# Herong1212/ORB_SLAM3_comments_ghr

Hardware: AMD Instinct MI355X
Metric: Mmatches/s (256-bit Hamming) (higher is better)
Workload: dtype fp4(e2m1)->f32; 1 GPU; C2: brute-force 256-bit Hamming top-2, 2000 x 2000 descriptors per frame, 1024 independent frames per launch per GPU (headline; the one-frame launch is `sing...; nq=2000, nt=2000, global_batch=1024, parallelism=replicas x1 (independent frames per GPU, no data-path collective)

## Files before the change

### orb_slam3_comments_ghr_amd/csrc/hamming_mfma.hip

```cpp
#include <algorithm>
#include <cstdlib>

#include "osg_internal.h"
#include "top2_key.h"

namespace {

typedef int i32x4 __attribute__((ext_vector_type(4)));
typedef int i32x16 __attribute__((ext_vector_type(16)));

constexpr int MF_PAD = 1 << 30;
constexpr int MF_RS = 272;

__device__ __forceinline__ int med3_i32(int a, int b, int c)
{
    return max(min(a, b), min(max(a, b), c));
}

__device__ __forceinline__ uint32_t spread_query(uint32_t nib)
{
    const uint32_t s = __umul24(nib, 0x204081u) & 0x01010101u;
    return ((0x80808080u - s) & 0x80808080u) | 0x40404040u;
}

__device__ __forceinline__ void key_push(int &k1, int &k2, int key)
{
    k2 = med3_i32(k1, key, k2);
    k1 = min(k1, key);
}

__device__ __forceinline__ void key_push2(int &k1, int &k2, int x, int y)
{
    const int m = med3_i32(k1, x, y);
    k1 = min(min(k1, x), y);
    k2 = min(m, k2);
}

__device__ __forceinline__ void key_push2f(int &k1, int &k2, int x, int y)
{
    const int m = __float_as_int(__builtin_amdgcn_fmed3f(__int_as_float(k1), __int_as_float(x), __int_as_float(y)));
    k1 = min(min(x, y), k1);
    k2 = min(m, k2);
}

__device__ __forceinline__ void key_merge(int &k1, int &k2, int a1, int a2)
{
    const int hi = max(k1, a1);
    k1 = min(k1, a1);
    k2 = min(min(k2, a2), hi);
}

template <int NW, int QT, int CR, int PIPE>
__global__ __launch_bounds__(NW * 64) void k_top2_mfma(const uint32_t *__restrict__ query, int nq,
                                                        const uint32_t *__restrict__ train, int nt,
                                                        int nqb, int32_t *__restrict__ out)
{
    constexpr int NT = NW * 64;
    constexpr int BPT = CR * 32 / NT;
    constexpr int WPT = BPT / 4;
    constexpr int TPR = 32 / BPT;
    constexpr int NTILE = CR / 32;
    static_assert(CR * 32 % NT == 0 && BPT % 4 == 0 && TPR >= 1, "chunk / workgroup shape");
    __shared__ __attribute__((aligned(16))) unsigned char s_buf[2 * CR * MF_RS];
    __shared__ uint2 s_lut[256];

    const int t = threadIdx.x, lane = t & 63;
    const int w = __builtin_amdgcn_readfirstlane(t >> 6);
    const int G = gridDim.x, L = blockIdx.x;
    const int logical = (G % 8 == 0) ? (L % 8) * (G / 8) + L / 8 : L;
    const int b = logical / nqb, qb = logical % nqb;
    const uint32_t *qf = query + (size_t)b * nq * 8;
    const uint32_t *tf = train + (size_t)b * nt * 8;
    int32_t *of = out + (size_t)b * nq * 3;

    for (int e = t; e < 256; e += NT) {
        uint32_t lo = 0, hi = 0;
#pragma unroll
        for (int y = 0; y < 4; y++) {
            lo |= ((e >> y) & 1u) << (8 * y + 7);
            hi |= ((e >> (y + 4)) & 1u) << (8 * y + 7);
        }
        s_lut[e] = make_uint2(lo, hi);
    }

    const int r = lane & 31, h = lane >> 5;
    const int qw0 = qb * (NW * QT * 32) + w * (QT * 32);
    const bool active = qw0 < nq;

    i32x4 bq[QT][8];
    int ka1[QT], ka2[QT], kb1[QT], kb2[QT], pq[QT];
#pragma unroll
    for (int j = 0; j < QT; j++) {
        const int q = min(qw0 + 32 * j + r, nq - 1);
        const uint4 lo = *(const uint4 *)(qf + (size_t)q * 8), hi = *(const uint4 *)(qf + (size_t)q * 8 + 4);
        const uint32_t wd[8] = {lo.x, lo.y, lo.z, lo.w, hi.x, hi.y, hi.z, hi.w};
        int pc = 0;
#pragma unroll
        for (int s = 0; s < 8; s++) {
            pc += __popc(wd[s]);
            const uint32_t hw = h ? (wd[s] >> 16) : (wd[s] & 0xFFFFu);
#pragma unroll
            for (int d = 0; d < 4; d++) bq[j][s][d] = (int)spread_query((hw >> (4 * d)) & 0xFu);
        }
        pq[j] = pc;
        ka1[j] = ka2[j] = kb1[j] = kb2[j] = (256 - pc) << MF_SHIFT;
    }
    i32x16 crow;
#pragma unroll
    for (int i = 0; i < 16; i++) crow[i] = (i & 3) + 8 * (i >> 2) + 4 * h;
    const int lbase = r * MF_RS + h * 16;

    const int erow = t / TPR, epart = t % TPR;
    auto load_chunk = [&](int c0, uint32_t (&pw)[WPT]) {
        const int row = c0 + erow;
        if (row < nt) {
            const uint32_t *src = tf + (size_t)row * 8 + epart * WPT;
#pragma unroll
            for (int i = 0; i < WPT; i += 2) {
                const uint2 v = *(const uint2 *)(src + i);
                pw[i] = v.x;
                pw[i + 1] = v.y;
            }
        } else {
#pragma unroll
            for (int i = 0; i < WPT; i++) pw[i] = 0u;
        }
    };
    auto store_chunk = [&](int buf, const uint32_t (&pw)[WPT]) {
        unsigned char *dst = s_buf + ((size_t)buf * CR + erow) * MF_RS;
#pragma unroll
        for (int i = 0; i < WPT; i++) {
#pragma unroll
            for (int hh = 0; hh < 2; hh++) {
                const int g = 2 * (epart * WPT + i) + hh;
                const uint2 v0 = s_lut[(pw[i] >> (16 * hh)) & 0xFFu];
                const uint2 v1 = s_lut[(pw[i] >> (16 * hh + 8)) & 0xFFu];
                *(i32x4 *)(dst + 16 * g) = i32x4{(int)v0.x, (int)v0.y, (int)v1.x, (int)v1.y};
            }
        }
    };

    auto frag = [&](const unsigned char *tb, int s) -> i32x4 { return *(const i32x4 *)(tb + lbase + 32 * s); };
    auto mfma = [&](const i32x4 &a, const i32x4 &bb, const i32x16 &c) {
        return __builtin_amdgcn_mfma_i32_32x32x32_i8(a, bb, c, 0, 0, 0);
    };
    auto epi = [&](const i32x16 (&acc)[QT]) {
#pragma unroll
        for (int j = 0; j < QT; j++) {
#pragma unroll
            for (int i = 0; i < 8; i += 2) {
                key_push2(ka1[j], ka2[j], acc[j][i], acc[j][i + 1]);
                key_push2(kb1[j], kb2[j], acc[j][i + 8], acc[j][i + 9]);
            }
            ka1[j] -= 32;
            ka2[j] -= 32;
            kb1[j] -= 32;
            kb2[j] -= 32;
        }
    };
    auto tile = [&](const unsigned char *tb, const i32x16 &cin) {
        i32x4 a[8];
#pragma unroll
        for (int s = 0; s < 8; s++) a[s] = frag(tb, s);
        i32x16 acc[QT];
#pragma unroll
        for (int j = 0; j < QT; j++) acc[j] = mfma(a[0], bq[j][0], cin);
#pragma unroll
        for (int s = 1; s < 8; s++)
#pragma unroll
            for (int j = 0; j < QT; j++) acc[j] = mfma(a[s], bq[j][s], acc[j]);
        epi(acc);
    };

    const int nch = (nt + CR - 1) / CR;
    {
        uint32_t pw[WPT];
        load_chunk(0, pw);
        __syncthreads();
        store_chunk(0, pw);
    }
    __syncthreads();
    for (int c = 0; c < nch; c++) {
        const int c0 = c * CR;
        uint32_t pw[WPT];
        const bool more = c + 1 < nch;
        if (more) load_chunk(c0 + CR, pw);
        if (active) {
            const unsigned char *sb = s_buf + (size_t)(c & 1) * CR * MF_RS;
            const int nfull = min(NTILE, (nt - c0) / 32);
            if (PIPE && nfull == NTILE) {
                i32x4 a[8];
                i32x16 accp[QT], acc[QT];
#pragma unroll
                for (int s = 0; s < 8; s++) a[s] = frag(sb, s);
#pragma unroll
                for (int s = 0; s < 8; s++) {
#pragma unroll
                    for (int j = 0; j < QT; j++) accp[j] = mfma(a[s], bq[j][s], s ? accp[j] : crow);
                    a[s] = frag(sb + 32 * MF_RS, s);
                    __builtin_amdgcn_sched_barrier(0);
                }
#pragma unroll
                for (int tt = 1; tt < NTILE; tt++) {
#pragma unroll
                    for (int s = 0; s < 8; s++) {
#pragma unroll
                        for (int j = 0; j < QT; j++) acc[j] = mfma(a[s], bq[j][s], s ? acc[j] : crow);
                        if (tt + 1 < NTILE) a[s] = frag(sb + (tt + 1) * 32 * MF_RS, s);
#pragma unroll
                        for (int j = 0; j < QT; j++) {
                            if (s & 1)
                                key_push2(kb1[j], kb2[j], accp[j][8 + (s & 6)], accp[j][9 + (s & 6)]);
                            else
                                key_push2(ka1[j], ka2[j], accp[j][s & 6], accp[j][1 + (s & 6)]);
                            if (s == 7) {
                                ka1[j] -= 32;
                                ka2[j] -= 32;
                                kb1[j] -= 32;
                                kb2[j] -= 32;
                            }
                        }
                        __builtin_amdgcn_sched_barrier(0);
                    }
#pragma unroll
                    for (int j = 0; j < QT; j++) accp[j] = acc[j];
                }
                epi(accp);
            } else {
#pragma unroll
                for (int tt = 0; tt < NTILE; tt++) {
                    if (tt >= nfull) break;
                    tile(sb + tt * 32 * MF_RS, crow);
                }
            }
            const int lim = nt - (c0 + nfull * 32);
            if (nfull < NTILE && lim > 0) {
                i32x16 cin;
#pragma unroll
                for (int i = 0; i < 16; i++) cin[i] = crow[i] + (crow[i] >= lim ? MF_PAD : 0);
                tile(sb + nfull * 32 * MF_RS, cin);
            }
        }
        if (more) store_chunk((c + 1) & 1, pw);
        __syncthreads();
    }
    if (!active) return;
    const int base = 32 * ((nt + 31) / 32);
#pragma unroll
    for (int j = 0; j < QT; j++) {
        int k1 = ka1[j], k2 = ka2[j];
        key_merge(k1, k2, kb1[j], kb2[j]);
        const int a1 = __shfl_xor(k1, 32), a2 = __shfl_xor(k2, 32);
        key_merge(k1, k2, a1, a2);
        const int q = qw0 + 32 * j + r;
        if (h == 0 && q < nq) {
            const int t1 = k1 + base, t2 = k2 + base;
            const int d1 = (t1 >> MF_SHIFT) + pq[j], d2 = (t2 >> MF_SHIFT) + pq[j];
            of[3 * q + 0] = d1 < 256 ? (t1 & (MF_MAX_ROWS - 1)) : -1;
            of[3 * q + 1] = min(d1, 256);
            of[3 * q + 2] = min(d2, 256);
        }
    }
}

constexpr int MX_RS = 144;
constexpr int MX_SCALE_TRAIN = 127 + 12;
constexpr int MX_SCALE_ONE = 127;
constexpr float MX_BIAS = 10485760.0f;
constexpr float MX_PAD = 1073741824.0f;

typedef int i32x8 __attribute__((ext_vector_type(8)));
typedef float f32x16 __attribute__((ext_vector_type(16)));

__device__ __forceinline__ uint32_t spread_nib(uint32_t x)
{
    x &= 0xFFu;
    x = (x | (x << 12)) & 0x000F000Fu;
    x = (x | (x << 6)) & 0x03030303u;
    return (x | (x << 3)) & 0x11111111u;
}

template <int NW, int QT, int CR, int PIPE>
__global__ __launch_bounds__(NW * 64) void k_top2_fp4(const uint32_t *__restrict__ query, int nq,
                                                       const uint32_t *__restrict__ train, int nt,
                                                       int nqb, int32_t *__restrict__ out)
{
    constexpr int NT = NW * 64;
    constexpr int BPT = CR * 32 / NT;
    constexpr int WPT = BPT / 4;
    constexpr int TPR = 32 / BPT;
    constexpr int NTILE = CR / 32;
    static_assert(CR * 32 % NT == 0 && BPT % 4 == 0 && TPR >= 1, "chunk / workgroup shape");
    __shared__ __attribute__((aligned(16))) unsigned char s_buf[2 * CR * MX_RS];
    __shared__ uint32_t s_lut[256];

    const int t = threadIdx.x, lane = t & 63;
    const int w = __builtin_amdgcn_readfirstlane(t >> 6);
    const int G = gridDim.x, L = blockIdx.x;
    const int logical = (G % 8 == 0) ? (L % 8) * (G / 8) + L / 8 : L;
    const int b = logical / nqb, qb = logical % nqb;
    const uint32_t *qf = query + (size_t)b * nq * 8;
    const uint32_t *tf = train + (size_t)b * nt * 8;
    int32_t *of = out + (size_t)b * nq * 3;

    for (int e = t; e < 256; e += NT) s_lut[e] = spread_nib((uint32_t)e) * 0xCu;

    const int r = lane & 31, h = lane >> 5;
    const int qw0 = qb * (NW * QT * 32) + w * (QT * 32);
    const bool active = qw0 < nq;

    i32x8 bq[QT][4];
    int ka1[QT], ka2[QT], kb1[QT], kb2[QT];
    constexpr bool ONE = PIPE == 3 || PIPE == 4 || PIPE == 5;
    constexpr bool PART = PIPE == 5;
    int(&kc1)[QT] = ONE ? ka1 : kb1;
    int(&kc2)[QT] = ONE ? ka2 : kb2;
    int pq[QT];
#pragma unroll
    for (int j = 0; j < QT; j++) {
        const int q = min(qw0 + 32 * j + r, nq - 1);
        const uint4 lo = *(const uint4 *)(qf + (size_t)q * 8), hi = *(const uint4 *)(qf + (size_t)q * 8 + 4);
        const uint32_t wd[8] = {lo.x, lo.y, lo.z, lo.w, hi.x, hi.y, hi.z, hi.w};
        int pc = 0;
#pragma unroll
        for (int k = 0; k < 8; k++) pc += __popc(wd[k]);
#pragma unroll
        for (int s = 0; s < 4; s++) {
            const uint32_t word = wd[2 * s + h];
#pragma unroll
            for (int d = 0; d < 4; d++)
                bq[j][s][d] = (int)(0x22222222u | ((~spread_nib(word >> (8 * d)) & 0x11111111u) << 3));
#pragma unroll
            for (int d = 4; d < 8; d++) bq[j][s][d] = 0;
        }
        pq[j] = pc;
        ka1[j] = ka2[j] = kb1[j] = kb2[j] = ((256 - pc) << MF_SHIFT) + MX_KEY0;
    }
    f32x16 crow;
#pragma unroll
    for (int i = 0; i < 16; i++) crow[i] = MX_BIAS + (float)((i & 3) + 8 * (i >> 2) + 4 * h);
    const int lbase = r * MX_RS + h * 16;

    const int erow = t / TPR, epart = t % TPR;
    auto load_chunk = [&](int c0, uint32_t (&pw)[WPT]) {
        const int row = c0 + erow;
        if (row < nt) {
            const uint32_t *src = tf + (size_t)row * 8 + epart * WPT;
#pragma unroll
            for (int i = 0; i < WPT; i += 2) {
                const uint2 v = *(const uint2 *)(src + i);
                pw[i] = v.x;
                pw[i + 1] = v.y;
            }
        } else {
#pragma unroll
            for (int i = 0; i < WPT; i++) pw[i] = 0u;
        }
    };
    auto store_chunk = [&](int buf, const uint32_t (&pw)[WPT]) {
        unsigned char *dst = s_buf + ((size_t)buf * CR + erow) * MX_RS;
#pragma unroll
        for (int i = 0; i < WPT; i++) {
            const uint32_t x = pw[i];
            *(i32x4 *)(dst + 16 * (epart * WPT + i)) =
                i32x4{(int)s_lut[x & 0xFFu], (int)s_lut[(x >> 8) & 0xFFu], (int)s_lut[(x >> 16) & 0xFFu],
                      (int)s_lut[x >> 24]};
        }
    };

    auto frag = [&](const unsigned char *tb, int s) -> i32x8 {
        const i32x4 v = *(const i32x4 *)(tb + lbase + 32 * s);
        return i32x8{v[0], v[1], v[2], v[3], 0, 0, 0, 0};
    };
    auto mfma = [&](const i32x8 &a, const i32x8 &bb, const f32x16 &c) {
        return __builtin_amdgcn_mfma_scale_f32_32x32x64_f8f6f4(a, bb, c, 4, 4, 0, MX_SCALE_TRAIN, 0, MX_SCALE_ONE);
    };
    auto epi = [&](const f32x16 (&acc)[QT]) {
#pragma unroll
        for (int j = 0; j < QT; j++) {
#pragma unroll
            for (int i = 0; i < 8; i += 2) {
                key_push2f(ka1[j], ka2[j], __float_as_int(acc[j][i]), __float_as_int(acc[j][i + 1]));
                key_push2f(kc1[j], kc2[j], __float_as_int(acc[j][i + 8]), __float_as_int(acc[j][i + 9]));
            }
            ka1[j] -= 32;
            ka2[j] -= 32;
            if (!ONE) {
                kb1[j] -= 32;
                kb2[j] -= 32;
            }
        }
    };
    auto tile = [&](const unsigned char *tb, const f32x16 &cin) {
        i32x8 a[4];
#pragma unroll
        for (int s = 0; s < 4; s++) a[s] = frag(tb, s);
        f32x16 acc[QT];
#pragma unroll
        for (int j = 0; j < QT; j++) acc[j] = mfma(a[0], bq[j][0], cin);
#pragma unroll
        for (int s = 1; s < 4; s++)
#pragma unroll
            for (int j = 0; j < QT; j++) acc[j] = mfma(a[s], bq[j][s], acc[j]);
        epi(acc);
    };

    const int nch = (nt + CR - 1) / CR;
    {
        uint32_t pw[WPT];
        load_chunk(0, pw);
        __syncthreads();
        store_chunk(0, pw);
    }
    __syncthreads();
    for (int c = 0; c < nch; c++) {
        const int c0 = c * CR;
        uint32_t pw[WPT];
        const bool more = c + 1 < nch;
        if (more) load_chunk(c0 + CR, pw);
        if (active) {
            const unsigned char *sb = s_buf + (size_t)(c & 1) * CR * MX_RS;
            const int nfull = min(NTILE, (nt - c0) / 32);
            if (PIPE && (nfull == NTILE || (PART && nfull >= 1))) {
                i32x8 a[4];
                f32x16 accp[QT], acc[QT];
#pragma unroll
                for (int s = 0; s < 4; s++) a[s] = frag(sb, s);
#pragma unroll
                for (int s = 0; s < 4; s++) {
#pragma unroll
                    for (int j = 0; j < QT; j++) accp[j] = mfma(a[s], bq[j][s], s ? accp[j] : crow);
                    a[s] = frag(sb + 32 * MX_RS, s);
                    __builtin_amdgcn_sched_barrier(0);
                }
#pragma unroll
                for (int tt = 1; tt < NTILE; tt++) {
                    if (PART && tt >= nfull) break;
#pragma unroll
                    for (int s = 0; s < 4; s++) {
#pragma unroll
                        for (int j = 0; j < QT; j++) acc[j] = mfma(a[s], bq[j][s], s ? acc[j] : crow);
                        if (tt + 1 < NTILE) a[s] = frag(sb + (tt + 1) * 32 * MX_RS, s);
                        if (PIPE == 4) {
                            if (s == 1) {
                                bool need = false;
#pragma unroll
                                for (int j = 0; j < QT; j++) {
                                    int m = __float_as_int(accp[j][0]);
#pragma unroll
                                    for (int e = 1; e < 16; e += 2)
                                        m = min(min(m, __float_as_int(accp[j][e])),
                                                __float_as_int(accp[j][e + 1 < 16 ? e + 1 : e]));
                                    need |= m < ka2[j];
                                }
                                if (__builtin_amdgcn_ballot_w64(need) != 0) {
#pragma unroll
                                    for (int j = 0; j < QT; j++)
#pragma unroll
                                        for (int e = 0; e < 16; e += 2)
                                            key_push2f(ka1[j], ka2[j], __float_as_int(accp[j][e]),
                                                      __float_as_int(accp[j][e + 1]));
                                }
#pragma unroll
                                for (int j = 0; j < QT; j++) {
                                    ka1[j] -= 32;
                                    ka2[j] -= 32;
                                }
                            }
                            __builtin_amdgcn_sched_barrier(0);
                            continue;
                        }
#pragma unroll
                        for (int j = 0; j < QT; j++) {
                            if (PIPE == 2) {
#pragma unroll
                                for (int p = 0; p < 8; p++) {
                                    if (p / 3 + 1 != s) continue;
                                    const int e = (p & 3) * 2 + (p >> 2) * 8;
                                    if (p < 4) key_push2f(ka1[j], ka2[j], __float_as_int(accp[j][e]), __float_as_int(accp[j][e + 1]));
                                    else key_push2f(kb1[j], kb2[j], __float_as_int(accp[j][e]), __float_as_int(accp[j][e + 1]));
                                }
                            } else {
                                key_push2f(ka1[j], ka2[j], __float_as_int(accp[j][2 * s]),
                                          __float_as_int(accp[j][2 * s + 1]));
                                key_push2f(kc1[j], kc2[j], __float_as_int(accp[j][8 + 2 * s]),
                                          __float_as_int(accp[j][9 + 2 * s]));
                            }
                            if (s == 3) {
                                ka1[j] -= 32;
                                ka2[j] -= 32;
                                if (!ONE) {
                                    kb1[j] -= 32;
                                    kb2[j] -= 32;
                                }
                            }
                        }
                        __builtin_amdgcn_sched_barrier(0);
                    }
#pragma unroll
                    for (int j = 0; j < QT; j++) accp[j] = acc[j];
                }
                epi(accp);
            } else {
#pragma unroll
                for (int tt = 0; tt < NTILE; tt++) {
                    if (tt >= nfull) break;
                    tile(sb + tt * 32 * MX_RS, crow);
                }
            }
            const int lim = nt - (c0 + nfull * 32);
            if (nfull < NTILE && lim > 0) {
                f32x16 cin;
#pragma unroll
                for (int i = 0; i < 16; i++)
                    cin[i] = crow[i] + ((i & 3) + 8 * (i >> 2) + 4 * h >= lim ? MX_PAD : 0.f);
                tile(sb + nfull * 32 * MX_RS, cin);
            }
        }
        if (more) store_chunk((c + 1) & 1, pw);
        __syncthreads();
    }
    if (!active) return;
    const int base = 32 * ((nt + 31) / 32);
#pragma unroll
    for (int j = 0; j < QT; j++) {
        int k1 = ka1[j], k2 = ka2[j];
        if (!ONE) key_merge(k1, k2, kb1[j], kb2[j]);
        const int a1 = __shfl_xor(k1, 32), a2 = __shfl_xor(k2, 32);
        key_merge(k1, k2, a1, a2);
        const int q = qw0 + 32 * j + r;
        if (h == 0 && q < nq) {
            const int t1 = k1 - MX_KEY0 + base, t2 = k2 - MX_KEY0 + base;
            const int d1 = (t1 >> MF_SHIFT) + pq[j], d2 = (t2 >> MF_SHIFT) + pq[j];
            of[3 * q + 0] = d1 < 256 ? (t1 & (MF_MAX_ROWS - 1)) : -1;
            of[3 * q + 1] = min(d1, 256);
            of[3 * q + 2] = min(d2, 256);
        }
    }
}

template <int NW, int QT, int CR>
__global__ __launch_bounds__(NW * 64) void k_top2_fp4p(const uint32_t *__restrict__ query, int nq,
                                                        const uint32_t *__restrict__ train, int nt,
                                                        int nqb, int n_items, int32_t *__restrict__ out)
{
    constexpr int NT = NW * 64;
    constexpr int BPT = CR * 32 / NT;
    constexpr int WPT = BPT / 4;
    constexpr int TPR = 32 / BPT;
    constexpr int NTILE = CR / 32;
    static_assert(CR * 32 % NT == 0 && BPT % 4 == 0 && TPR >= 1, "chunk / workgroup shape");
    __shared__ __attribute__((aligned(16))) unsigned char s_buf[2 * CR * MX_RS];
    __shared__ uint32_t s_lut[256];

    const int t = threadIdx.x, lane = t & 63;
    const int w = __builtin_amdgcn_readfirstlane(t >> 6);
    const int G = gridDim.x;
    auto logical_of = [&](int item) { return (n_items % 8 == 0) ? (item % 8) * (n_items / 8) + item / 8 : item; };
    int item = blockIdx.x;
    if (item >= n_items) return;
    for (int e = t; e < 256; e += NT) s_lut[e] = spread_nib((uint32_t)e) * 0xCu;
    const int r = lane & 31, h = lane >> 5;
    const int lbase = r * MX_RS + h * 16;
    const int erow = t / TPR, epart = t % TPR;
    auto load_chunk = [&](const uint32_t *tfp, int c0, uint32_t (&pw)[WPT]) {
        const int row = c0 + erow;
        if (row < nt) {
            const uint32_t *src = tfp + (size_t)row * 8 + epart * WPT;
#pragma unroll
            for (int i = 0; i < WPT; i += 2) {
                const uint2 v = *(const uint2 *)(src + i);
                pw[i] = v.x;
                pw[i + 1] = v.y;
            }
        } else {
#pragma unroll
            for (int i = 0; i < WPT; i++) pw[i] = 0u;
        }
    };
    auto store_chunk = [&](int buf, const uint32_t (&pw)[WPT]) {
        unsigned char *dst = s_buf + ((size_t)buf * CR + erow) * MX_RS;
#pragma unroll
        for (int i = 0; i < WPT; i++) {
            const uint32_t x = pw[i];
            *(i32x4 *)(dst + 16 * (epart * WPT + i)) =
                i32x4{(int)s_lut[x & 0xFFu], (int)s_lut[(x >> 8) & 0xFFu], (int)s_lut[(x >> 16) & 0xFFu],
                      (int)s_lut[x >> 24]};
        }
    };
    auto frag = [&](const unsigned char *tb, int s) -> i32x8 {
        const i32x4 v = *(const i32x4 *)(tb + lbase + 32 * s);
        return i32x8{v[0], v[1], v[2], v[3], 0, 0, 0, 0};
    };
    auto mfma = [&](const i32x8 &a, const i32x8 &bb, const f32x16 &c) {
        return __builtin_amdgcn_mfma_scale_f32_32x32x64_f8f6f4(a, bb, c, 4, 4, 0, MX_SCALE_TRAIN, 0, MX_SCALE_ONE);
    };
    const int nch = (nt + CR - 1) / CR;
    {
        uint32_t pw[WPT];
        load_chunk(train + (size_t)(logical_of(item) / nqb) * nt * 8, 0, pw);
        __syncthreads();
        store_chunk(0, pw);
    }
    __syncthreads();
    int bufbase = 0;
    for (; item < n_items; item += G) {
        const int logical = logical_of(item);
        const int b = logical / nqb, qb = logical % nqb;
        const uint32_t *qf = query + (size_t)b * nq * 8;
        const uint32_t *tf = train + (size_t)b * nt * 8;
        int32_t *of = out + (size_t)b * nq * 3;
        const int next = item + G;
        const uint32_t *tfn = next < n_items ? train + (size_t)(logical_of(next) / nqb) * nt * 8 : nullptr;
        const int qw0 = qb * (NW * QT * 32) + w * (QT * 32);
        const bool active = qw0 < nq;
        i32x8 bq[QT][4];
        int ka1[QT], ka2[QT], pq[QT];
#pragma unroll
        for (int j = 0; j < QT; j++) {
            const int q = min(qw0 + 32 * j + r, nq - 1);
            const uint4 lo = *(const uint4 *)(qf + (size_t)q * 8), hi = *(const uint4 *)(qf + (size_t)q * 8 + 4);
            const uint32_t wd[8] = {lo.x, lo.y, lo.z, lo.w, hi.x, hi.y, hi.z, hi.w};
            int pc = 0;
#pragma unroll
            for (int k = 0; k < 8; k++) pc += __popc(wd[k]);
#pragma unroll
            for (int s = 0; s < 4; s++) {
                const uint32_t word = wd[2 * s + h];
#pragma unroll
                for (int d = 0; d < 4; d++)
                    bq[j][s][d] = (int)(0x22222222u | ((~spread_nib(word >> (8 * d)) & 0x11111111u) << 3));
#pragma unroll
                for (int d = 4; d < 8; d++) bq[j][s][d] = 0;
            }
            pq[j] = pc;
            ka1[j] = ka2[j] = ((256 - pc) << MF_SHIFT) + MX_KEY0;
        }
        f32x16 crow;
#pragma unroll
        for (int i = 0; i < 16; i++) crow[i] = MX_BIAS + (float)((i & 3) + 8 * (i >> 2) + 4 * h);
        auto epi = [&](const f32x16 (&acc)[QT]) {
#pragma unroll
            for (int j = 0; j < QT; j++) {
#pragma unroll
                for (int i = 0; i < 8; i += 2) {
                    key_push2f(ka1[j], ka2[j], __float_as_int(acc[j][i]), __float_as_int(acc[j][i + 1]));
                    key_push2f(ka1[j], ka2[j], __float_as_int(acc[j][i + 8]), __float_as_int(acc[j][i + 9]));
                }
                ka1[j] -= 32;
                ka2[j] -= 32;
            }
        };
        auto tile = [&](const unsigned char *tb, const f32x16 &cin) {
            i32x8 a[4];
#pragma unroll
            for (int s = 0; s < 4; s++) a[s] = frag(tb, s);
            f32x16 acc[QT];
#pragma unroll
            for (int j = 0; j < QT; j++) acc[j] = mfma(a[0], bq[j][0], cin);
#pragma unroll
            for (int s = 1; s < 4; s++)
#pragma unroll
                for (int j = 0; j < QT; j++) acc[j] = mfma(a[s], bq[j][s], acc[j]);
            epi(acc);
        };
        for (int c = 0; c < nch; c++) {
            const int c0 = c * CR;
            uint32_t pw[WPT];
            const bool more_in = c + 1 < nch, more = more_in || tfn != nullptr;
            if (more_in) load_chunk(tf, c0 + CR, pw);
            else if (tfn) load_chunk(tfn, 0, pw);
            if (active) {
                const unsigned char *sb = s_buf + (size_t)((c + bufbase) & 1) * CR * MX_RS;
                const int nfull = min(NTILE, (nt - c0) / 32);
                if (nfull == NTILE) {
                    i32x8 a[4];
                    f32x16 accp[QT], acc[QT];
#pragma unroll
                    for (int s = 0; s < 4; s++) a[s] = frag(sb, s);
#pragma unroll
                    for (int s = 0; s < 4; s++) {
#pragma unroll
                        for (int j = 0; j < QT; j++) accp[j] = mfma(a[s], bq[j][s], s ? accp[j] : crow);
                        a[s] = frag(sb + 32 * MX_RS, s);
                        __builtin_amdgcn_sched_barrier(0);
                    }
#pragma unroll
                    for (int tt = 1; tt < NTILE; tt++) {
#pragma unroll
                        for (int s = 0; s < 4; s++) {
#pragma unroll
                            for (int j = 0; j < QT; j++) acc[j] = mfma(a[s], bq[j][s], s ? acc[j] : crow);
                            if (tt + 1 < NTILE) a[s] = frag(sb + (tt + 1) * 32 * MX_RS, s);
#pragma unroll
                            for (int j = 0; j < QT; j++) {
                                key_push2f(ka1[j], ka2[j], __float_as_int(accp[j][2 * s]),
                                           __float_as_int(accp[j][2 * s + 1]));
                                key_push2f(ka1[j], ka2[j], __float_as_int(accp[j][8 + 2 * s]),
                                           __float_as_int(accp[j][9 + 2 * s]));
                                if (s == 3) {
                                    ka1[j] -= 32;
                                    ka2[j] -= 32;
                                }
                            }
                            __builtin_amdgcn_sched_barrier(0);
                        }
#pragma unroll
                        for (int j = 0; j < QT; j++) accp[j] = acc[j];
                    }
                    epi(accp);
                } else {
#pragma unroll
                    for (int tt = 0; tt < NTILE; tt++) {
                        if (tt >= nfull) break;
                        tile(sb + tt * 32 * MX_RS, crow);
                    }
                }
                const int lim = nt - (c0 + nfull * 32);
                if (nfull < NTILE && lim > 0) {
                    f32x16 cin;
#pragma unroll
                    for (int i = 0; i < 16; i++)
                        cin[i] = crow[i] + ((i & 3) + 8 * (i >> 2) + 4 * h >= lim ? MX_PAD : 0.f);
                    tile(sb + nfull * 32 * MX_RS, cin);
                }
            }
            if (more) store_chunk((c + 1 + bufbase) & 1, pw);
            __syncthreads();
        }
        bufbase = (bufbase + nch) & 1;
        if (active) {
            const int base = 32 * ((nt + 31) / 32);
#pragma unroll
            for (int j = 0; j < QT; j++) {
                int k1 = ka1[j], k2 = ka2[j];
                const int a1 = __shfl_xor(k1, 32), a2 = __shfl_xor(k2, 32);
                key_merge(k1, k2, a1, a2);
                const int q = qw0 + 32 * j + r;
                if (h == 0 && q < nq) {
                    const int t1 = k1 - MX_KEY0 + base, t2 = k2 - MX_KEY0 + base;
                    const int d1 = (t1 >> MF_SHIFT) + pq[j], d2 = (t2 >> MF_SHIFT) + pq[j];
                    of[3 * q + 0] = d1 < 256 ? (t1 & (MF_MAX_ROWS - 1)) : -1;
                    of[3 * q + 1] = min(d1, 256);
                    of[3 * q + 2] = min(d2, 256);
                }
            }
        }
    }
}

template <int NW, int CR>
__global__ __launch_bounds__(NW * 64) void k_top2_fp4q2(const uint32_t *__restrict__ query, int nq,
                                                         const uint32_t *__restrict__ train, int nt,
                                                         int nqb, int32_t *__restrict__ out)
{
    constexpr int NT = NW * 64;
    constexpr int BPT = CR * 32 / NT;
    constexpr int WPT = BPT / 4;
    constexpr int TPR = 32 / BPT;
    constexpr int NTILE = CR / 32;
    static_assert(CR * 32 % NT == 0 && BPT % 8 == 0 && TPR >= 1, "chunk / workgroup shape");
    __shared__ __attribute__((aligned(16))) unsigned char s_buf[2 * CR * MX_RS];
    __shared__ uint32_t s_lut[256];

    const int t = threadIdx.x, lane = t & 63;
    const int w = __builtin_amdgcn_readfirstlane(t >> 6);
    const int G = gridDim.x, L = blockIdx.x;
    const int logical = (G % 8 == 0) ? (L % 8) * (G / 8) + L / 8 : L;
    const int b = logical / nqb, qb = logical % nqb;
    const uint32_t *qf = query + (size_t)b * nq * 8;
    const uint32_t *tf = train + (size_t)b * nt * 8;
    int32_t *of = out + (size_t)b * nq * 3;

    for (int e = t; e < 256; e += NT) s_lut[e] = spread_nib((uint32_t)e) * 0xCu;

    const int r = lane & 31, h = lane >> 5;
    const int qw0 = qb * (NW * 64) + w * 64;
    const bool act0 = qw0 < nq, act1 = qw0 + 32 < nq;

    i32x8 bq[2][4];
    int k1[2], k2[2];
#pragma unroll
    for (int j = 0; j < 2; j++) {
        const int q = min(qw0 + 32 * j + r, nq - 1);
        const uint4 lo = *(const uint4 *)(qf + (size_t)q * 8), hi = *(const uint4 *)(qf + (size_t)q * 8 + 4);
        const uint32_t wd[8] = {lo.x, lo.y, lo.z, lo.w, hi.x, hi.y, hi.z, hi.w};
        int pc = 0;
#pragma unroll
        for (int k = 0; k < 8; k++) pc += __popc(wd[k]);
#pragma unroll
        for (int s = 0; s < 4; s++) {
            const uint32_t word = wd[2 * s + h];
#pragma unroll
            for (int d = 0; d < 4; d++)
                bq[j][s][d] = (int)(0x22222222u | ((~spread_nib(word >> (8 * d)) & 0x11111111u) << 3));
#pragma unroll
            for (int d = 4; d < 8; d++) bq[j][s][d] = 0;
        }
        k1[j] = k2[j] = ((256 - pc) << MF_SHIFT) + MX_KEY0;
    }
    f32x16 crow;
#pragma unroll
    for (int i = 0; i < 16; i++) crow[i] = MX_BIAS + (float)((i & 3) + 8 * (i >> 2) + 4 * h);
    const int lbase = r * MX_RS + h * 16;

    auto load_chunk = [&](int c0, uint32_t (&pw)[WPT]) {
        if (c0 + t / TPR < nt) {
            const char *src = (const char *)tf + (unsigned)((c0 * 8 + t * WPT) * 4);
#pragma unroll
            for (int i = 0; i < WPT; i += 2) {
                const uint2 v = *(const uint2 *)(src + 4 * i);
                pw[i] = v.x;
                pw[i + 1] = v.y;
            }
        } else {
#pragma unroll
            for (int i = 0; i < WPT; i++) pw[i] = 0u;
        }
    };
    auto store_chunk = [&](int buf, const uint32_t (&pw)[WPT]) {
        unsigned char *dst = s_buf + buf * (CR * MX_RS) + (t / TPR) * MX_RS + (t % TPR) * (16 * WPT);
#pragma unroll
        for (int i = 0; i < WPT; i++) {
            const uint32_t x = pw[i];
            *(i32x4 *)(dst + 16 * i) =
                i32x4{(int)s_lut[x & 0xFFu], (int)s_lut[(x >> 8) & 0xFFu], (int)s_lut[(x >> 16) & 0xFFu],
                      (int)s_lut[x >> 24]};
        }
    };
    auto frag = [&](const unsigned char *tb, int s) -> i32x8 {
        const i32x4 v = *(const i32x4 *)(tb + lbase + 32 * s);
        return i32x8{v[0], v[1], v[2], v[3], 0, 0, 0, 0};
    };
    auto mfma = [&](const i32x8 &a, const i32x8 &bb, const f32x16 &c) {
        return __builtin_amdgcn_mfma_scale_f32_32x32x64_f8f6f4(a, bb, c, 4, 4, 0, MX_SCALE_TRAIN, 0, MX_SCALE_ONE);
    };
    auto push = [&](int j, const f32x16 &acc, int s) {
        key_push2f(k1[j], k2[j], __float_as_int(acc[2 * s]), __float_as_int(acc[2 * s + 1]));
        key_push2f(k1[j], k2[j], __float_as_int(acc[8 + 2 * s]), __float_as_int(acc[9 + 2 * s]));
        if (s == 3) k1[j] -= TOP2_TILE_ROWS;
    };
    auto pushk = [&](int j, const f32x16 &acc, int s) {
        const int lo = s == 0 ? 0 : 3 * (s - 1), hi = s == 0 ? 0 : (s == 3 ? 8 : 3 * s);
#pragma unroll
        for (int p = lo; p < hi; p++) {
            const int e = (p & 1) * 8 + 2 * (p >> 1);
            key_push2f(k1[j], k2[j], __float_as_int(acc[e]), __float_as_int(acc[e + 1]));
        }
        if (s == 3) k1[j] -= TOP2_TILE_ROWS;
    };
    auto tile = [&](const unsigned char *tb, const f32x16 &cin) {
        i32x8 a[4];
#pragma unroll
        for (int s = 0; s < 4; s++) a[s] = frag(tb, s);
        f32x16 acc0 = mfma(a[0], bq[0][0], cin);
#pragma unroll
        for (int s = 1; s < 4; s++) acc0 = mfma(a[s], bq[0][s], acc0);
        if (act1) {
            f32x16 acc1 = mfma(a[0], bq[1][0], cin);
#pragma unroll
            for (int s = 1; s < 4; s++) acc1 = mfma(a[s], bq[1][s], acc1);
#pragma unroll
            for (int s = 0; s < 4; s++) push(0, acc0, s);
#pragma unroll
            for (int s = 0; s < 4; s++) push(1, acc1, s);
        } else {
#pragma unroll
            for (int s = 0; s < 4; s++) push(0, acc0, s);
        }
    };

    const int nch = (nt + CR - 1) / CR;
    {
        uint32_t pw[WPT];
        load_chunk(0, pw);
        __syncthreads();
        store_chunk(0, pw);
    }
    __syncthreads();
    for (int c = 0; c < nch; c++) {
        const int c0 = c * CR;
        uint32_t pw[WPT];
        const bool more = c + 1 < nch;
        if (more) load_chunk(c0 + CR, pw);
        if (act0) {
            const unsigned char *sb = s_buf + (size_t)(c & 1) * CR * MX_RS;
            const int nfull = min(NTILE, (nt - c0) / 32);
            if (act1 && nfull == NTILE) {
                i32x8 a[4];
                f32x16 acc0, acc1;
#pragma unroll
                for (int s = 0; s < 4; s++) a[s] = frag(sb, s);
#pragma unroll
                for (int s = 0; s < 4; s++) {
                    acc0 = mfma(a[s], bq[0][s], s ? acc0 : crow);
                    __builtin_amdgcn_sched_barrier(0);
                }
#pragma unroll
                for (int tt = 0; tt < NTILE; tt++) {
#pragma unroll
                    for (int s = 0; s < 4; s++) {
                        acc1 = mfma(a[s], bq[1][s], s ? acc1 : crow);
                        if (tt + 1 < NTILE) a[s] = frag(sb + (tt + 1) * 32 * MX_RS, s);
                        __builtin_amdgcn_sched_barrier(0);
                        pushk(0, acc0, s);
                        __builtin_amdgcn_sched_barrier(0);
                    }
                    if (tt + 1 == NTILE) break;
#pragma unroll
                    for (int s = 0; s < 4; s++) {
                        acc0 = mfma(a[s], bq[0][s], s ? acc0 : crow);
                        __builtin_amdgcn_sched_barrier(0);
                        pushk(1, acc1, s);
                        __builtin_amdgcn_sched_barrier(0);
                    }
                }
#pragma unroll
                for (int s = 0; s < 4; s++) push(1, acc1, s);
            } else {
#pragma unroll 1
                for (int tt = 0; tt < nfull; tt++) tile(sb + tt * 32 * MX_RS, crow);
            }
            const int lim = nt - (c0 + nfull * 32);
            if (nfull < NTILE && lim > 0) {
                f32x16 cin;
#pragma unroll
                for (int i = 0; i < 16; i++)
                    cin[i] = crow[i] + (4 * h >= lim - ((i & 3) + 8 * (i >> 2)) ? MX_PAD : 0.f);
                tile(sb + nfull * 32 * MX_RS, cin);
            }
        }
        if (more) store_chunk((c + 1) & 1, pw);
        __syncthreads();
    }
    if (!act0) return;
    const int base = 32 * ((nt + 31) / 32);
    const int lane_end = (int)__builtin_amdgcn_mbcnt_hi(~0u, __builtin_amdgcn_mbcnt_lo(~0u, 0u));
#pragma unroll
    for (int j = 0; j < 2; j++) {
        int m1 = k1[j], m2 = k2[j];
        const int a1 = __shfl_xor(m1, 32), a2 = __shfl_xor(m2, 32);
        m2 = min(min(m2, a2), max(m1, a1) + TOP2_K2_LAST_REBASE);
        m1 = min(m1, a1);
        const int q = qw0 + 32 * j + lane_end;
        if (lane_end < 32 && q < nq) {
            const uint4 lo = *(const uint4 *)(qf + (size_t)q * 8), hi = *(const uint4 *)(qf + (size_t)q * 8 + 4);
            const int pc = __popc(lo.x) + __popc(lo.y) + __popc(lo.z) + __popc(lo.w) + __popc(hi.x) + __popc(hi.y) +
                           __popc(hi.z) + __popc(hi.w);
            const int d1 = top2_k1_dist(m1, base) + pc, d2 = top2_k2_dist(m2) + pc;
            of[3 * q + 0] = d1 < 256 ? top2_k1_row(m1, base) : -1;
            of[3 * q + 1] = min(d1, 256);
            of[3 * q + 2] = min(d2, 256);
        }
    }
}

template <int NW, int CR>
int launch_fp4q2(osg_ctx *ctx, const void *d_query, int nq, const void *d_train, int nt, int nb, void *d_out)
{
    const int nqb = (nq + NW * 64 - 1) / (NW * 64);
    const long long g = (long long)nqb * nb;
    OSG_REQUIRE(ctx, g <= 0x7FFFFFFF, "grid too large");
    hipLaunchKernelGGL((k_top2_fp4q2<NW, CR>), dim3((unsigned)g), dim3(NW * 64), 0, ctx->stream,
                       (const uint32_t *)d_query, nq, (const uint32_t *)d_train, nt, nqb, (int32_t *)d_out);
    OSG_HIP_CHECK(ctx, hipGetLastError());
    return OSG_OK;
}

template <int NW, int QT, int CR>
int launch_fp4p(osg_ctx *ctx, const void *d_query, int nq, const void *d_train, int nt, int nb, void *d_out)
{
    const int nqb = (nq + NW * QT * 32 - 1) / (NW * QT * 32);
    const long long items = (long long)nqb * nb;
    OSG_REQUIRE(ctx, items <= 0x7FFFFFFF, "grid too large");
    static int ncu = 0;
    if (ncu == 0) {
        int dev = 0, n = 0;
        if (hipGetDevice(&dev) == hipSuccess && hipDeviceGetAttribute(&n, hipDeviceAttributeMultiprocessorCount, dev) == hipSuccess && n > 0)
            ncu = n;
        else
            ncu = 256;
    }
    const int g = (int)std::min<long long>(items, ncu);
    hipLaunchKernelGGL((k_top2_fp4p<NW, QT, CR>), dim3((unsigned)std::max(g, 1)), dim3(NW * 64), 0, ctx->stream,
                       (const uint32_t *)d_query, nq, (const uint32_t *)d_train, nt, nqb, (int)items, (int32_t *)d_out);
    OSG_HIP_CHECK(ctx, hipGetLastError());
    return OSG_OK;
}

template <int NW, int QT, int CR, int PIPE>
int launch_fp4(osg_ctx *ctx, const void *d_query, int nq, const void *d_train, int nt, int nb, void *d_out)
{
    const int nqb = (nq + NW * QT * 32 - 1) / (NW * QT * 32);
    const long long g = (long long)nqb * nb;
    OSG_REQUIRE(ctx, g <= 0x7FFFFFFF, "grid too large");
    hipLaunchKernelGGL((k_top2_fp4<NW, QT, CR, PIPE>), dim3((unsigned)g), dim3(NW * 64), 0, ctx->stream,
                       (const uint32_t *)d_query, nq, (const uint32_t *)d_train, nt, nqb, (int32_t *)d_out);
    OSG_HIP_CHECK(ctx, hipGetLastError());
    return OSG_OK;
}

template <int NW, int QT, int CR, int PIPE>
int launch(osg_ctx *ctx, const void *d_query, int nq, const void *d_train, int nt, int nb, void *d_out)
{
    const int nqb = (nq + NW * QT * 32 - 1) / (NW * QT * 32);
    const long long g = (long long)nqb * nb;
    OSG_REQUIRE(ctx, g <= 0x7FFFFFFF, "grid too large");
    hipLaunchKernelGGL((k_top2_mfma<NW, QT, CR, PIPE>), dim3((unsigned)g), dim3(NW * 64), 0, ctx->stream,
                       (const uint32_t *)d_query, nq, (const uint32_t *)d_train, nt, nqb, (int32_t *)d_out);
    OSG_HIP_CHECK(ctx, hipGetLastError());
    return OSG_OK;
}

}

int osg_top2_mfma_max_rows() { return MF_MAX_ROWS; }

namespace {
int mfma_shape()
{
    static const int shape = getenv("OSG_TOP2_MFMA_SHAPE") ? atoi(getenv("OSG_TOP2_MFMA_SHAPE")) : 0;
    return shape;
}
bool mfma_fp4()
{
    static const bool fp4 = !(getenv("OSG_TOP2_FP4") && atoi(getenv("OSG_TOP2_FP4")) == 0);
    return fp4;
}
void mfma_shape_of(bool fp4, int shape, int *d)
{
    static const int i8[5][4] = {{16, 1, 256, 1}, {8, 2, 256, 1}, {16, 1, 256, 0}, {8, 2, 256, 0}, {8, 1, 256, 1}};
    static const int f4[14][4] = {{16, 1, 256, 3}, {8, 2, 256, 1}, {16, 1, 256, 0}, {16, 1, 256, 3}, {8, 1, 256, 1},
                                  {16, 2, 256, 1}, {16, 1, 256, 2}, {16, 1, 256, 1}, {16, 1, 256, 4}, {8, 1, 256, 3},
                                  {16, 1, 512, 3}, {16, 1, 256, 5}, {16, 1, 512, 5}, {16, 1, 256, 6}};
    const int *s = fp4 ? f4[(shape >= 1 && shape <= 13 && shape != 3) ? shape : 0]
                       : i8[(shape >= 1 && shape <= 4) ? shape : 0];
    for (int i = 0; i < 4; i++) d[i] = s[i];
}
bool mfma_q2(bool fp4, int shape) { return fp4 && !(shape >= 1 && shape <= 13); }
}

int osg_hamming_top2_batch_plan(osg_ctx *ctx, int32_t nq, int32_t nt, int32_t nb, char *name, int32_t len)
{
    if (!ctx || !name || len <= 0) return OSG_E_INVALID;
    const bool mf = getenv("OSG_TOP2_BATCH_MFMA") == nullptr || atoi(getenv("OSG_TOP2_BATCH_MFMA")) != 0;
    if (nq <= 0 || nb <= 0 || nt <= 0 || !mf || nt > MF_MAX_ROWS) {
        snprintf(name, (size_t)len, "%s", nq <= 0 || nb <= 0 ? "none" : "k_top2_batch");
        return OSG_OK;
    }
    if (mfma_q2(mfma_fp4(), mfma_shape())) {
        snprintf(name, (size_t)len, "k_top2_fp4q2<16,256> grid=%lld x %d", (long long)((nq + 1023) / 1024) * nb, 1024);
        return OSG_OK;
    }
    int d[4];
    mfma_shape_of(mfma_fp4(), mfma_shape(), d);
    const int per_wg = d[0] * d[1] * 32;
    snprintf(name, (size_t)len, "%s<%d,%d,%d,%d> grid=%lld x %d", mfma_fp4() ? "k_top2_fp4" : "k_top2_mfma", d[0], d[1],
             d[2], d[3], (long long)((nq + per_wg - 1) / per_wg) * nb, d[0] * 64);
    return OSG_OK;
}

int osg_launch_top2_batch_mfma(osg_ctx *ctx, const void *d_query, int32_t nq, const void *d_train, int32_t nt,
                               int32_t nb, void *d_out)
{
    OSG_REQUIRE(ctx, nt >= 1 && nt <= MF_MAX_ROWS, "nt=%d outside the MFMA path's 1..%d rows", nt, MF_MAX_ROWS);
    const int shape = mfma_shape();
    if (mfma_fp4()) {
        if (mfma_q2(true, shape)) return launch_fp4q2<16, 256>(ctx, d_query, nq, d_train, nt, nb, d_out);
        switch (shape) {
        case 1: return launch_fp4<8, 2, 256, 1>(ctx, d_query, nq, d_train, nt, nb, d_out);
        case 2: return launch_fp4<16, 1, 256, 0>(ctx, d_query, nq, d_train, nt, nb, d_out);
        case 4: return launch_fp4<8, 1, 256, 1>(ctx, d_query, nq, d_train, nt, nb, d_out);
        case 5: return launch_fp4<16, 2, 256, 1>(ctx, d_query, nq, d_train, nt, nb, d_out);
        case 6: return launch_fp4<16, 1, 256, 2>(ctx, d_query, nq, d_train, nt, nb, d_out);
        case 7: return launch_fp4<16, 1, 256, 1>(ctx, d_query, nq, d_train, nt, nb, d_out);
        case 8: return launch_fp4<16, 1, 256, 4>(ctx, d_query, nq, d_train, nt, nb, d_out);
        case 9: return launch_fp4<8, 1, 256, 3>(ctx, d_query, nq, d_train, nt, nb, d_out);
        case 10: return launch_fp4<16, 1, 512, 3>(ctx, d_query, nq, d_train, nt, nb, d_out);
        case 11: return launch_fp4<16, 1, 256, 5>(ctx, d_query, nq, d_train, nt, nb, d_out);
        case 12: return launch_fp4<16, 1, 512, 5>(ctx, d_query, nq, d_train, nt, nb, d_out);
        case 13: return launch_fp4p<16, 1, 256>(ctx, d_query, nq, d_train, nt, nb, d_out);
        default: return launch_fp4<16, 1, 256, 3>(ctx, d_query, nq, d_train, nt, nb, d_out);
        }
    }
    switch (shape) {
    case 1: return launch<8, 2, 256, 1>(ctx, d_query, nq, d_train, nt, nb, d_out);
    case 2: return launch<16, 1, 256, 0>(ctx, d_query, nq, d_train, nt, nb, d_out);
    case 3: return launch<8, 2, 256, 0>(ctx, d_query, nq, d_train, nt, nb, d_out);
    case 4: return launch<8, 1, 256, 1>(ctx, d_query, nq, d_train, nt, nb, d_out);
    default: return launch<16, 1, 256, 1>(ctx, d_query, nq, d_train, nt, nb, d_out);
    }
}
```

Before: 10.69 million Mmatches/s.

## Replace double-buffered train staging with three-slot LDS ring and cross-chunk MFMA pipeline

Swaps the two-buffer shared-memory staging of train descriptors for a three-slot ring that prefetches two chunks ahead. Global loads are issued before query setup, and the store/load for future chunks happens at a single barrier seam per chunk. The MFMA/top-2 push software pipeline now continues across chunk boundaries instead of draining at each one. It also adds a cheaper multiply-based nibble spread for the LUT and query fragments. In exchange it uses more LDS, which may lower occupancy, and adds complex barrier and slot bookkeeping along with inline asm to recompute lane ids.

```diff
diff --git a/orb_slam3_comments_ghr_amd/csrc/hamming_mfma.hip b/orb_slam3_comments_ghr_amd/csrc/hamming_mfma.hip
--- a/orb_slam3_comments_ghr_amd/csrc/hamming_mfma.hip
+++ b/orb_slam3_comments_ghr_amd/csrc/hamming_mfma.hip
@@ -3,6 +3,7 @@
 
 #include "osg_internal.h"
 #include "top2_key.h"
+#include "top2_ring.h"
 
 namespace {
 
@@ -278,6 +279,13 @@
     x = (x | (x << 12)) & 0x000F000Fu;
     x = (x | (x << 6)) & 0x03030303u;
     return (x | (x << 3)) & 0x11111111u;
+}
+
+__device__ __forceinline__ uint32_t spread_nib9(uint32_t x)
+{
+    uint32_t lo3 = x * 0x40201u;
+    asm("" : "+v"(lo3));
+    return (lo3 | (x << 27)) & 0x88888888u;
 }
 
 template <int NW, int QT, int CR, int PIPE>
@@ -760,8 +768,10 @@
     constexpr int TPR = 32 / BPT;
     constexpr int NTILE = CR / 32;
     static_assert(CR * 32 % NT == 0 && BPT % 8 == 0 && TPR >= 1, "chunk / workgroup shape");
-    __shared__ __attribute__((aligned(16))) unsigned char s_buf[2 * CR * MX_RS];
-    __shared__ uint32_t s_lut[256];
+    constexpr int SLOTB = CR * MX_RS;
+    __shared__ __attribute__((aligned(16))) unsigned char s_mem[1024 + TOP2_RING_SLOTS * SLOTB];
+    uint32_t *const s_lut = (uint32_t *)s_mem;
+    unsigned char *const s_buf = s_mem + 1024;
 
     const int t = threadIdx.x, lane = t & 63;
     const int w = __builtin_amdgcn_readfirstlane(t >> 6);
@@ -772,28 +782,43 @@
     const uint32_t *tf = train + (size_t)b * nt * 8;
     int32_t *of = out + (size_t)b * nq * 3;
 
-    for (int e = t; e < 256; e += NT) s_lut[e] = spread_nib((uint32_t)e) * 0xCu;
+    for (int e = t; e < 256; e += NT) {
+        const uint32_t x = spread_nib9((uint32_t)e);
+        s_lut[e] = x | (x >> 1);
+    }
 
     const int r = lane & 31, h = lane >> 5;
     const int qw0 = qb * (NW * 64) + w * 64;
     const bool act0 = qw0 < nq, act1 = qw0 + 32 < nq;
 
+    auto load_chunk = [&](int t, int c0, uint32_t (&pw)[WPT]) {
+        const char *src = (const char *)tf + (c0 + t / TPR < nt ? (unsigned)((c0 * 8 + t * WPT) * 4) : 0u);
+#pragma unroll
+        for (int i = 0; i < WPT; i += 2) {
+            const uint2 v = *(const uint2 *)(src + 4 * i);
+            pw[i] = v.x;
+            pw[i + 1] = v.y;
+        }
+    };
+    uint32_t pw[WPT], p1[WPT];
+    load_chunk(t, 0, pw);
+    load_chunk(t, CR, p1);
+
     i32x8 bq[2][4];
     int k1[2], k2[2];
 #pragma unroll
     for (int j = 0; j < 2; j++) {
         const int q = min(qw0 + 32 * j + r, nq - 1);
         const uint4 lo = *(const uint4 *)(qf + (size_t)q * 8), hi = *(const uint4 *)(qf + (size_t)q * 8 + 4);
-        const uint32_t wd[8] = {lo.x, lo.y, lo.z, lo.w, hi.x, hi.y, hi.z, hi.w};
-        int pc = 0;
-#pragma unroll
-        for (int k = 0; k < 8; k++) pc += __popc(wd[k]);
+        const int pc = __popc(lo.x) + __popc(lo.y) + __popc(lo.z) + __popc(lo.w) + __popc(hi.x) + __popc(hi.y) +
+                       __popc(hi.z) + __popc(hi.w);
+        const uint32_t wsel[4] = {h ? lo.y : lo.x, h ? lo.w : lo.z, h ? hi.y : hi.x, h ? hi.w : hi.z};
 #pragma unroll
         for (int s = 0; s < 4; s++) {
-            const uint32_t word = wd[2 * s + h];
+            const uint32_t word = wsel[s];
 #pragma unroll
             for (int d = 0; d < 4; d++)
-                bq[j][s][d] = (int)(0x22222222u | ((~spread_nib(word >> (8 * d)) & 0x11111111u) << 3));
+                bq[j][s][d] = (int)(spread_nib9((word >> (8 * d)) & 0xFFu) ^ 0xAAAAAAAAu);
 #pragma unroll
             for (int d = 4; d < 8; d++) bq[j][s][d] = 0;
         }
@@ -802,27 +827,14 @@
     f32x16 crow;
 #pragma unroll
     for (int i = 0; i < 16; i++) crow[i] = MX_BIAS + (float)((i & 3) + 8 * (i >> 2) + 4 * h);
-    const int lbase = r * MX_RS + h * 16;
-
-    auto load_chunk = [&](int c0, uint32_t (&pw)[WPT]) {
-        if (c0 + t / TPR < nt) {
-            const char *src = (const char *)tf + (unsigned)((c0 * 8 + t * WPT) * 4);
-#pragma unroll
-            for (int i = 0; i < WPT; i += 2) {
-                const uint2 v = *(const uint2 *)(src + 4 * i);
-                pw[i] = v.x;
-                pw[i + 1] = v.y;
-            }
-        } else {
-#pragma unroll
-            for (int i = 0; i < WPT; i++) pw[i] = 0u;
-        }
-    };
-    auto store_chunk = [&](int buf, const uint32_t (&pw)[WPT]) {
-        unsigned char *dst = s_buf + buf * (CR * MX_RS) + (t / TPR) * MX_RS + (t % TPR) * (16 * WPT);
+    int lbase = r * MX_RS + h * 16;
+
+    auto store_chunk = [&](int t, int buf, int c0, const uint32_t (&pw)[WPT]) {
+        const bool in = c0 + t / TPR < nt;
+        unsigned char *dst = s_buf + buf * SLOTB + ((t & (NT - 1)) / TPR) * MX_RS + (t % TPR) * (16 * WPT);
 #pragma unroll
         for (int i = 0; i < WPT; i++) {
-            const uint32_t x = pw[i];
+            const uint32_t x = in ? pw[i] : 0u;
             *(i32x4 *)(dst + 16 * i) =
                 i32x4{(int)s_lut[x & 0xFFu], (int)s_lut[(x >> 8) & 0xFFu], (int)s_lut[(x >> 16) & 0xFFu],
                       (int)s_lut[x >> 24]};
@@ -870,38 +882,53 @@
         }
     };
 
-    const int nch = (nt + CR - 1) / CR;
-    {
-        uint32_t pw[WPT];
-        load_chunk(0, pw);
+    const int nch = top2_ring_chunks(nt, CR), nfc = top2_ring_full_chunks(nt, CR);
+    __syncthreads();
+    store_chunk(t, top2_ring_slot(0), 0, pw);
+    store_chunk(t, top2_ring_slot(1), CR, p1);
+    load_chunk(t, TOP2_RING_AHEAD * CR, pw);
+    __syncthreads();
+    auto lane_again = [&]() {
+        int ln;
+        asm volatile("v_mbcnt_lo_u32_b32 %0, -1, 0\n\tv_mbcnt_hi_u32_b32 %0, -1, %0" : "=v"(ln));
+        return ln & 63;
+    };
+    auto seam = [&](int c, int freed) {
         __syncthreads();
-        store_chunk(0, pw);
-    }
-    __syncthreads();
-    for (int c = 0; c < nch; c++) {
-        const int c0 = c * CR;
-        uint32_t pw[WPT];
-        const bool more = c + 1 < nch;
-        if (more) load_chunk(c0 + CR, pw);
-        if (act0) {
-            const unsigned char *sb = s_buf + (size_t)(c & 1) * CR * MX_RS;
-            const int nfull = min(NTILE, (nt - c0) / 32);
-            if (act1 && nfull == NTILE) {
-                i32x8 a[4];
-                f32x16 acc0, acc1;
-#pragma unroll
-                for (int s = 0; s < 4; s++) a[s] = frag(sb, s);
+        const int ln = lane_again(), tv = w * 64 + ln;
+        store_chunk(tv, freed, (c + TOP2_RING_AHEAD) * CR, pw);
+        load_chunk(tv, (c + TOP2_RING_AHEAD + 1) * CR, pw);
+        return ln;
+    };
+    int slot = top2_ring_slot(0), freed = top2_ring_slot(TOP2_RING_SLOTS - 1);
+    if (act1) {
+        if (nfc > 0) {
+            i32x8 a[4];
+            f32x16 acc0, acc1;
+#pragma unroll
+            for (int s = 0; s < 4; s++) a[s] = frag(s_buf + slot * SLOTB, s);
+#pragma unroll
+            for (int i = 0; i < 16; i++) acc1[i] = MX_PAD;
+            k1[1] += TOP2_TILE_ROWS;
+            for (int c = 0; c < nfc; c++) {
 #pragma unroll
                 for (int s = 0; s < 4; s++) {
                     acc0 = mfma(a[s], bq[0][s], s ? acc0 : crow);
                     __builtin_amdgcn_sched_barrier(0);
+                    pushk(1, acc1, s);
+                    __builtin_amdgcn_sched_barrier(0);
                 }
+                const int ln = seam(c, freed);
+                const int next = top2_ring_next(slot);
+                lbase = (ln & 31) * MX_RS + (ln >> 5) * 16;
+                const unsigned char *sb = s_buf + slot * SLOTB, *sn = sb + (next - slot) * SLOTB;
 #pragma unroll
                 for (int tt = 0; tt < NTILE; tt++) {
+                    const unsigned char *nb = tt + 1 < NTILE ? sb + (tt + 1) * 32 * MX_RS : sn;
 #pragma unroll
                     for (int s = 0; s < 4; s++) {
                         acc1 = mfma(a[s], bq[1][s], s ? acc1 : crow);
-                        if (tt + 1 < NTILE) a[s] = frag(sb + (tt + 1) * 32 * MX_RS, s);
+                        a[s] = frag(nb, s);
                         __builtin_amdgcn_sched_barrier(0);
                         pushk(0, acc0, s);
                         __builtin_amdgcn_sched_barrier(0);
@@ -915,14 +942,35 @@
                         __builtin_amdgcn_sched_barrier(0);
                     }
                 }
-#pragma unroll
-                for (int s = 0; s < 4; s++) push(1, acc1, s);
-            } else {
+                freed = slot;
+                slot = next;
+            }
+#pragma unroll
+            for (int s = 0; s < 4; s++) push(1, acc1, s);
+        }
+    } else {
+        for (int c = 0; c < nfc; c++) {
+            seam(c, freed);
+            if (act0) {
+                const int nfull = min(NTILE, (nt - c * CR) / 32);
 #pragma unroll 1
-                for (int tt = 0; tt < nfull; tt++) tile(sb + tt * 32 * MX_RS, crow);
-            }
+                for (int tt = 0; tt < nfull; tt++) tile(s_buf + slot * SLOTB + tt * 32 * MX_RS, crow);
+            }
+            freed = slot;
+            slot = top2_ring_next(slot);
+        }
+    }
+    if (nfc < nch) {
+        seam(nfc, freed);
+        if (act0) {
+            const int ln = (int)__builtin_amdgcn_mbcnt_hi(~0u, __builtin_amdgcn_mbcnt_lo(~0u, 0u)), h = ln >> 5;
+            lbase = (ln & 31) * MX_RS + h * 16;
+            const unsigned char *sb = s_buf + slot * SLOTB;
+            const int c0 = nfc * CR, nfull = (nt - c0) / 32;
+#pragma unroll 1
+            for (int tt = 0; tt < nfull; tt++) tile(sb + tt * 32 * MX_RS, crow);
             const int lim = nt - (c0 + nfull * 32);
-            if (nfull < NTILE && lim > 0) {
+            if (lim > 0) {
                 f32x16 cin;
 #pragma unroll
                 for (int i = 0; i < 16; i++)
@@ -930,8 +978,6 @@
                 tile(sb + nfull * 32 * MX_RS, cin);
             }
         }
-        if (more) store_chunk((c + 1) & 1, pw);
-        __syncthreads();
     }
     if (!act0) return;
     const int base = 32 * ((nt + 31) / 32);
diff --git a/orb_slam3_comments_ghr_amd/csrc/top2_ring.h b/orb_slam3_comments_ghr_amd/csrc/top2_ring.h
--- /dev/null
+++ b/orb_slam3_comments_ghr_amd/csrc/top2_ring.h
@@ -0,0 +1,24 @@
+#pragma once
+
+constexpr int TOP2_RING_SLOTS = 3;
+constexpr int TOP2_RING_AHEAD = 2;
+constexpr int TOP2_RING_PROLOGUE_BARRIERS = 2;
+
+constexpr int top2_ring_slot(int chunk, int slots = TOP2_RING_SLOTS) { return chunk % slots; }
+constexpr int top2_ring_next(int slot, int slots = TOP2_RING_SLOTS) { return slot + 1 == slots ? 0 : slot + 1; }
+
+constexpr int top2_ring_chunks(int nt, int cr) { return (nt + cr - 1) / cr; }
+constexpr int top2_ring_full_chunks(int nt, int cr) { return nt / cr; }
+constexpr int top2_ring_barriers(int nt, int cr) { return TOP2_RING_PROLOGUE_BARRIERS + top2_ring_chunks(nt, cr); }
+
+constexpr int top2_ring_prologue_store_epoch() { return 1; }
+constexpr int top2_ring_block_epoch(int c) { return TOP2_RING_PROLOGUE_BARRIERS + 1 + c; }
+constexpr int top2_ring_write_epoch(int chunk)
+{
+    return chunk < TOP2_RING_AHEAD ? top2_ring_prologue_store_epoch() : top2_ring_block_epoch(chunk - TOP2_RING_AHEAD);
+}
+constexpr int top2_ring_first_read_epoch(int chunk)
+{
+    return chunk == 0 ? TOP2_RING_PROLOGUE_BARRIERS : top2_ring_block_epoch(chunk - 1);
+}
+constexpr int top2_ring_last_read_epoch(int chunk) { return top2_ring_block_epoch(chunk); }
```

Result: faster. 10.90 million Mmatches/s, median of 6 (+1.9%).
